# whatshap/whatshap

Measured on AMD Instinct MI355X. Metric: variant-columns/sec at max-coverage 20 (bipartition-costs/sec reported alongside), higher is better.
Workload: dtype u32; 1 GPU; synthetic diploid single-individual, max-coverage 20: 1 block of 200000 SNVs (BASELINE configs[2]); blocks=1, blocks_in_flight_per_gpu=1, tables_per_launch=1, max_coverage=20, optimal_cost_checksum=1611545, rendezvous=none

## Files before the change

whatshap_amd/csrc/dp_device.hip:

```cpp
#include <hip/hip_runtime.h>

#include <algorithm>
#include <atomic>
#include <cctype>
#include <chrono>
#include <cstdio>
#include <cstdlib>
#include <cstring>
#include <mutex>
#include <string>
#include <vector>

#include "debug_build.h"
#ifdef WHAMD_DEBUG_BUILD
#include "../../include/whatshap_amd_debug.h"
#endif
#include "device_runtime.h"
#include "device_table.h"
#include "genotype.h"
#include "table_plan.h"

namespace whamd {

namespace {
// ... 1567 lines not shown
		return WHAMD_OK;
	}
};

whamd_status_t DeviceTable::enqueue_group(DeviceTable* const* tables, const Problem* const* problems, Solution* const* solutions, size_t n_tables, std::string& msg) {
	if (n_tables == 0) return WHAMD_OK;
	HIP_TRY(hipSetDevice(tables[0]->impl_->device));
	Impl::GroupSubmission g(tables, problems, solutions, n_tables, msg);
	whamd_status_t st = g.open_members();
	if (st != WHAMD_OK) return st;
	const auto t_submit0 = std::chrono::steady_clock::now();
	for (size_t k = 0; k < g.max_steps; ++k) {
		g.add_super_step(k);
		for (int v = 0; v < GROUP_VARIANTS; ++v) g.flush((GroupVariant)v);
		if ((st = g.submit_singles(k)) != WHAMD_OK) return st;
	}
	if (getenv("WHAMD_DEBUG_TIMING"))
		fprintf(stderr, "[whamd timing] group of %zu tables in 1 part(s): %zu super-steps submitted in %.2f ms (host)\n", n_tables, g.max_steps,
		        std::chrono::duration<double, std::milli>(std::chrono::steady_clock::now() - t_submit0).count());
	if ((st = g.mark_forward_end()) != WHAMD_OK) return st;
	if ((st = g.walk_back()) != WHAMD_OK) return st;
	return g.submit_tails();
}

void DeviceTable::wait_last_of_each_stream(DeviceTable* const* tables, size_t n_tables) {
	std::vector<std::pair<hipStream_t, const Impl*>> last;
	for (size_t i = 0; i < n_tables; ++i) {
		const Impl& m = *tables[i]->impl_;
		if (!m.inflight.tail_elsewhere || !m.ev3) continue;
		bool found = false;
		for (auto& e : last) {
			if (e.first != m.inflight.tail_stream || e.second->device != m.device) continue;
			found = true;
			if (m.inflight.tail_seq > e.second->inflight.tail_seq) e.second = &m;
		}
		if (!found) last.emplace_back(m.inflight.tail_stream, &m);
	}
	for (const auto& e : last) {
		if (hipSetDevice(e.second->device) != hipSuccess || hipEventSynchronize(e.second->ev3) != hipSuccess) (void)hipGetLastError();
	}
}

void DeviceTable::read_timing(whamd_solve_stats& st) {
	Impl& m = *impl_;
	if (!m.inflight.timing_pending) return;
	m.inflight.timing_pending = false;
	if (hipSetDevice(m.device) != hipSuccess) return;
	float f01 = 0, f12 = 0, f03 = 0;
	if (hipEventElapsedTime(&f01, m.ev0, m.ev1) != hipSuccess || hipEventElapsedTime(&f12, m.ev1, m.ev2) != hipSuccess || hipEventElapsedTime(&f03, m.ev0, m.ev3) != hipSuccess) {
		(void)hipGetLastError();
		return;
	}
	st.forward_ms = f01;
	st.backtrace_ms = f12;
	st.total_ms = f03;
}

whamd_status_t DeviceTable::Impl::report_slot_stamps(std::string& msg) const {
	const Impl& m = *this;
	if (m.dev.dp.dbg_flags & 256u) return m.report_slot_wave_stamps(msg);
	std::vector<unsigned long long> d(m.tp.splan.runs.size() * 48);
	HIP_TRY(hipMemcpy(d.data(), m.dev.dp.dbg, d.size() * 8, hipMemcpyDeviceToHost));
	double a[6] = {0, 0, 0, 0, 0, 0};
	double percol[32] = {0};
	size_t cnt = 0;
	for (size_t i = 0; i < m.tp.splan.runs.size(); ++i) {
		if (m.tp.splan.runs[i].ncols != 22 || d[48 * i + 5] == 0) continue;
		for (int k = 0; k < 6; ++k) a[k] += (double)d[48 * i + k];
		for (int k = 0; k < 22; ++k) percol[k] += (double)d[48 * i + 8 + k];
		++cnt;
	}
	if (cnt) fprintf(stderr, "[whamd slot stamps] %zu runs, wave 0 of workgroup 0, shader cycles: prologue issue %.0f, loads landed %.0f, column loop %.0f (%.1f per column, %.1f columns), exit %.0f\n",
	                 cnt, a[0] / cnt, a[1] / cnt, a[2] / cnt, a[2] / std::max(a[4], 1.0), a[4] / cnt, a[3] / cnt);
	if (cnt) {
		fprintf(stderr, "[whamd slot stamps] cycles after the loop start at which column c had its cost added:");
		for (int k = 0; k < 22; ++k) fprintf(stderr, " %.0f", percol[k] / cnt);
		fprintf(stderr, "\n");
	}
	return WHAMD_OK;
}

whamd_status_t DeviceTable::Impl::report_slot_wave_stamps(std::string& msg) const {
	const Impl& m = *this;
	constexpr int NW = 8, NS = 8;
	static const char* const names[NS] = {"wave start", "entering cells requested", "last prologue request", "entering cells landed", "all landed, loop starts",
	                                      "first wave-slot ending reached", "first wave-slot ending left", "loop end"};
	static const int word[NS] = {0, 1, 2, 3, 7, 4, 5, 6};
	const size_t nruns = m.tp.splan.runs.size(), per_run = (size_t)SLOT_WAVE_STAMP_WGS * SLOT_WAVE_STAMP_WORDS;
	std::vector<unsigned long long> d(nruns * per_run);
	HIP_TRY(hipMemcpy(d.data(), m.dev.dp.dbg + m.dev.dp.dbg_wg_off + SLOT_WAVE_STAMP_OFF, d.size() * 8, hipMemcpyDeviceToHost));
	for (uint32_t sel = 0; sel < SLOT_WAVE_STAMP_WGS; ++sel) {
		double mean[NS][NW] = {}, spread[NS] = {}, spread_max[NS] = {}, lat_rank[NW] = {}, req_rank[NW] = {}, land_rank[NW] = {};
		size_t last[2][NW] = {}, cnt = 0;
		for (size_t i = 0; i < nruns; ++i) {
			const unsigned long long* r = d.data() + i * per_run + sel * SLOT_WAVE_STAMP_WORDS;
			bool full = m.tp.splan.runs[i].ncols == 22;
			for (int v = 0; v < NW; ++v) full = full && r[v * 8 + 6] != 0 && r[v * 8 + 4] != 0;
			if (!full) continue;
			unsigned long long s0 = r[0];
			for (int v = 1; v < NW; ++v) s0 = std::min(s0, r[v * 8]);
			double at[NS][NW];
			for (int k = 0; k < NS; ++k) {
				double lo = 1e300, hi = 0;
				int hi_at = 0;
				for (int v = 0; v < NW; ++v) {
					at[k][v] = (double)(r[v * 8] - s0) + (k ? (double)r[v * 8 + word[k]] : 0.0);
					mean[k][v] += at[k][v];
					lo = std::min(lo, at[k][v]);
					if (at[k][v] > hi) { hi = at[k][v]; hi_at = v; }
				}
				spread[k] += hi - lo;
				spread_max[k] = std::max(spread_max[k], hi - lo);
				if (k == 3) last[0][hi_at]++;
				if (k == 5) last[1][hi_at]++;
			}
			int order[NW];
			for (int v = 0; v < NW; ++v) order[v] = v;
			std::sort(order, order + NW, [&](int a, int b) { return at[1][a] < at[1][b]; });
			for (int q = 0; q < NW; ++q) { req_rank[q] += at[1][order[q]]; land_rank[q] += at[3][order[q]]; lat_rank[q] += at[3][order[q]] - at[1][order[q]]; }
			++cnt;
		}
		if (!cnt) continue;
		fprintf(stderr, "[whamd slot wave stamps] workgroup %u: %zu runs of 22 columns, shader cycles after the workgroup's earliest wave start; waves 0 .. 7 | mean spread, largest spread\n", 3 * sel, cnt);
		for (int k = 0; k < NS; ++k) {
			fprintf(stderr, "[whamd slot wave stamps]   %-31s", names[k]);
			for (int v = 0; v < NW; ++v) fprintf(stderr, " %6.0f", mean[k][v] / cnt);
			fprintf(stderr, " | %6.0f %6.0f\n", spread[k] / cnt, spread_max[k]);
		}
		for (int h = 0; h < 2; ++h) {
			fprintf(stderr, "[whamd slot wave stamps]   runs in which wave v is the last %-14s", h ? "at the ending:" : "to have cells:");
			for (int v = 0; v < NW; ++v) fprintf(stderr, " %6zu", last[h][v]);
			fprintf(stderr, "\n");
		}
		fprintf(stderr, "[whamd slot wave stamps]   by the order of the waves' requests -- requested:     ");
		for (int q = 0; q < NW; ++q) fprintf(stderr, " %6.0f", req_rank[q] / cnt);
		fprintf(stderr, "\n[whamd slot wave stamps]                                           landed:        ");
		for (int q = 0; q < NW; ++q) fprintf(stderr, " %6.0f", land_rank[q] / cnt);
		fprintf(stderr, "\n[whamd slot wave stamps]                                           latency:       ");
		for (int q = 0; q < NW; ++q) fprintf(stderr, " %6.0f", lat_rank[q] / cnt);
		fprintf(stderr, "\n");
	}
	return WHAMD_OK;
}

whamd_status_t DeviceTable::Impl::report_resident_stamps(std::string& msg) const {
	const Impl& m = *this;
	std::vector<unsigned long long> d(m.tp.plan.segments.size() * 8);
	HIP_TRY(hipMemcpy(d.data(), m.dev.dp.dbg, d.size() * 8, hipMemcpyDeviceToHost));
	unsigned long long a = 0, b = 0, c2 = 0, cols = 0, p1 = 0, p2 = 0, p3 = 0, ns = 0;
	for (size_t i = 0; i < m.tp.plan.segments.size(); ++i) { a += d[8 * i]; b += d[8 * i + 1]; c2 += d[8 * i + 2]; cols += d[8 * i + 3]; p1 += d[8 * i + 4]; p2 += d[8 * i + 5]; p3 += d[8 * i + 6]; ns += d[8 * i + 7]; }
	if (!m.tp.plan.ped_columns.empty() || (m.dev.dp.dbg_flags & 4u))
		fprintf(stderr, "[whamd timing] run prologue (wave 0 of workgroup 0), cycles after the first instruction: kernel arguments usable %.0f, first loaded data %.0f, everything staged %.0f\n",
		        (double)p2 / std::max<unsigned long long>(ns, 1), (double)p3 / std::max<unsigned long long>(ns, 1), (double)p1 / std::max<unsigned long long>(ns, 1));
	else
	fprintf(stderr, "[whamd timing] per barrier step (wave 0 of workgroup 0, %.1f steps per run): hot words %.0f, evaluate %.0f, barrier %.0f cycles\n",
	        (double)ns / m.tp.plan.segments.size(), (double)p1 / std::max<unsigned long long>(ns, 1), (double)p2 / std::max<unsigned long long>(ns, 1), (double)p3 / std::max<unsigned long long>(ns, 1));
	{
		unsigned long long b3[6] = {0, 0, 0, 0, 0, 0};
		HIP_TRY(hipMemcpy(b3, m.dev.dp.dbg + m.dev.dp.dbg_wg_off + 4 * 512 * 2, sizeof b3, hipMemcpyDeviceToHost));
		if (b3[2]) fprintf(stderr, "[whamd timing] backtrace per run: record load + prefetch %.0f cycles, walk + hand-over %.0f cycles (%llu runs); of the latter: local exit index %.0f, chain %.0f, logical indices + stores %.0f\n",
		                   (double)b3[0] / b3[2], (double)b3[1] / b3[2], b3[2], (double)b3[3] / b3[2], (double)b3[4] / b3[2], (double)b3[5] / b3[2]);
	}
	if (m.tp.plan.segments.size() > 104) {
		std::vector<unsigned long long> wg(4 * 512 * 2);
		HIP_TRY(hipMemcpy(wg.data(), m.dev.dp.dbg + m.dev.dp.dbg_wg_off, wg.size() * 8, hipMemcpyDeviceToHost));
		unsigned long long prev_end = 0;
		for (int sgi = 0; sgi < 4; ++sgi) {
			const uint32_t G = 1u << m.tp.plan.segments[100 + sgi].g;
			unsigned long long s0 = ~0ull, s1 = 0, e0 = ~0ull, e1 = 0;
			for (uint32_t ww = 0; ww < G; ++ww) {
				const unsigned long long a2 = wg[((size_t)sgi * 512 + ww) * 2], b2 = wg[((size_t)sgi * 512 + ww) * 2 + 1];
				s0 = std::min(s0, a2); s1 = std::max(s1, a2); e0 = std::min(e0, b2); e1 = std::max(e1, b2);
			}
			fprintf(stderr, "[whamd timing] run %d (%u workgroups): first start +%.2f us after previous run's last end; starts spread %.2f us; first end %.2f us, last end %.2f us after first start\n",
			        100 + sgi, G, prev_end ? (double)(s0 - prev_end) / 100.0 : 0.0, (double)(s1 - s0) / 100.0, (double)(e0 - s0) / 100.0, (double)(e1 - s0) / 100.0);
			prev_end = e1;
		}
	}
	float f01 = 0;
	(void)hipEventElapsedTime(&f01, m.ev0, m.ev1);
	fprintf(stderr, "[whamd timing] segments %zu cols %llu | cycles/segment: prologue %.0f columns %.0f (%.0f per column) store %.0f | fwd %.3f ms, %.2f us per segment\n",
	        m.tp.plan.segments.size(), cols, (double)a / m.tp.plan.segments.size(), (double)b / m.tp.plan.segments.size(),
	        (double)b / std::max<unsigned long long>(cols, 1), (double)c2 / m.tp.plan.segments.size(), f01, f01 * 1e3 / m.tp.plan.segments.size());
	return WHAMD_OK;
}

whamd_status_t DeviceTable::wait(const Problem& p, Solution& s, whamd_solve_stats& st, std::string& msg) {
	Impl& m = *impl_;
	if (p.n_cols == 0) return WHAMD_OK;
	HIP_TRY(hipSetDevice(m.device));
	const uint64_t launches = m.inflight.launches;
	if (m.inflight.tail_elsewhere) HIP_TRY(hipEventSynchronize(m.ev3));
	else { HIP_TRY(hipStreamSynchronize(m.stream)); m.own_stream_used = false; }
	m.upload_pending = false;
	m.give_preview_block();
	const uint32_t n = p.n_cols;
	std::memcpy(s.path_index.data(), m.dev.h_pinned, (size_t)n * 4);
// ... 202 lines not shown
```

whatshap_amd/csrc/kernels_slots.h:

```cpp

__device__ __forceinline__ uint32_t slot_cost(uint32_t A, uint32_t K, uint32_t Cc) { return min(min(A, K - A), Cc); }

template <int LR, int J>
__device__ __forceinline__ uint32_t slot_end_reg(uint32_t (&D)[1 << LR], uint32_t qthr, uint32_t qmask) {
	constexpr int R = 1 << LR;
	uint32_t takes = 0;
#pragma unroll
	for (int r0 = 0; r0 < R; ++r0) {
		if (r0 & (1 << J)) continue;
		const int r1 = r0 | (1 << J);
		const uint32_t q0 = qthr ^ ((qmask >> r0) & 1u), q1 = qthr ^ ((qmask >> r1) & 1u);
		const uint32_t a = D[r0], b = D[r1];
		takes |= (b < a + q0) ? (1u << r0) : 0u;
		takes |= (a < b + q1) ? (1u << r1) : 0u;
		D[r0] = D[r1] = min(a, b);
	}
	return takes;
}

template <int LR>
__device__ __forceinline__ uint32_t slot_end_partner(uint32_t (&D)[1 << LR], const uint32_t (&other)[1 << LR], uint32_t qthr, uint32_t qmask) {
	constexpr int R = 1 << LR;
	uint32_t takes = 0;
#pragma unroll
// ... 407 lines not shown
	"s_lshl_b32 %[sa], 1, %[sl]\n\t"                \
	"v_xor_b32_e32 %[a], %[sa], %[l4]\n\t"                                                                             \
	"ds_bpermute_b32 v60, %[a], %[d0]\n\t"                                                                             \
	"ds_bpermute_b32 v61, %[a], %[d1]\n\t"                                                                             \
	"ds_bpermute_b32 v62, %[a], %[d2]\n\t"                                                                             \
	"ds_bpermute_b32 v63, %[a], %[d3]\n\t"                                                                             \
	"s_branch .Lxm%=\n"                                                                                                \
	".Lxw%=:\n\t"                                   \
	"s_sub_u32 %[sa], %[sl], 8\n\t"                                                                                    \
	"s_lshl_b32 %[sa], 0x400, %[sa]\n\t"                                                                               \
	"s_bfe_u32 %[sl], %[cw], 0x1000f\n\t"           \
	"s_mul_i32 %[sl], %[sl], %[xby]\n\t"                                                                               \
	"v_mov_b32_e32 v56, %[d0]\n\t"                                                                                     \
	"v_mov_b32_e32 v57, %[d1]\n\t"                                                                                     \
	"v_mov_b32_e32 v58, %[d2]\n\t"                                                                                     \
	"v_mov_b32_e32 v59, %[d3]\n\t"                                                                                     \
	"v_add_u32_e32 %[a], %[sl], %[t16]\n\t"                                                                            \
	"ds_write_b128 %[a], v[56:59]\n\t"                                                                                 \
	"v_xor_b32_e32 %[a], %[sa], %[t16]\n\t"                                                                            \
	"v_add_u32_e32 %[a], %[sl], %[a]\n\t"                                                                              \
	"s_waitcnt lgkmcnt(0)\n\t"                                                                                         \
	"s_barrier\n\t"                                                                                                    \
	"ds_read_b128 v[60:63], %[a]\n\t"                                                                                  \
	"s_branch .Lxm%=\n"                                                                                                \
	".Lxr%=:\n\t"                                               \
	"s_cmp_eq_u32 %[sl], 0\n\t"                                                                                        \
	"s_cbranch_scc0 .Lxq%=\n\t"                                                                                        \
	"v_mov_b32_e32 v60, %[d1]\n\t"                                                                                     \
	"v_mov_b32_e32 v61, %[d0]\n\t"                                                                                     \
	"v_mov_b32_e32 v62, %[d3]\n\t"                                                                                     \
	"v_mov_b32_e32 v63, %[d2]\n\t"                                                                                     \
	"s_branch .Lxm%=\n"                                                                                                \
	".Lxq%=:\n\t"                                                                                                      \
	"v_mov_b32_e32 v60, %[d2]\n\t"                                                                                     \
	"v_mov_b32_e32 v61, %[d3]\n\t"                                                                                     \
	"v_mov_b32_e32 v62, %[d0]\n\t"                                                                                     \
	"v_mov_b32_e32 v63, %[d1]\n"                                                                                       \
	".Lxm%=:\n\t"                                   \
	"v_and_b32_e32 %[t], 1, %[par]\n\t"                                                                                \
	"v_cmp_ne_u32_e64 %[qt], 0, %[t]\n\t"                                                                              \
	"v_lshrrev_b32_e32 %[par], 1, %[par]\n\t"                             \
	"s_not_b64 %[qn], %[qt]\n\t"                                                                                       \
	"s_bitcmp1_b32 %[cw], 8\n\t"                     \
	"s_cselect_b64 %[q1], %[qn], %[qt]\n\t"                                                                            \
	"s_bitcmp1_b32 %[cw], 9\n\t"                                                                                       \
	"s_cselect_b64 %[q2], %[qn], %[qt]\n\t"                                                                            \
	"s_bitcmp1_b32 %[cw], 10\n\t"                                                                                      \
	"s_cselect_b64 %[q3], %[qn], %[qt]\n\t"                                                                            \
	"s_waitcnt lgkmcnt(0)\n\t"                                                                                         \
	"v_subb_co_u32_e64 %[t], %[q3], %[d3], v63, %[q3]\n\t"                                                                     \
	"v_subb_co_u32_e64 %[t], %[q2], %[d2], v62, %[q2]\n\t"                                                             \
	"v_subb_co_u32_e64 %[t], %[q1], %[d1], v61, %[q1]\n\t"                                                             \
	"v_subb_co_u32_e64 %[t], %[qt], %[d0], v60, %[qt]\n\t"                                                             \
	"v_cndmask_b32_e64 %[tk], 0, 1, %[q3]\n\t"                                                                         \
	"v_max_u32_e32 %[d3], %[d3], v63\n\t"                                                                              \
	"v_addc_co_u32_e64 %[tk], %[qn], %[tk], %[tk], %[q2]\n\t"                                                          \
	"v_max_u32_e32 %[d2], %[d2], v62\n\t"                                                                              \
	"v_addc_co_u32_e64 %[tk], %[qn], %[tk], %[tk], %[q1]\n\t"                                                          \
	"v_max_u32_e32 %[d1], %[d1], v61\n\t"                                                                              \
	"v_addc_co_u32_e64 %[tk], %[qn], %[tk], %[tk], %[qt]\n\t"                                                          \
	"v_max_u32_e32 %[d0], %[d0], v60\n\t"                                                                              \
	"global_store_byte %[ro], %[tk], %[rb]\n\t"     \
	"v_add_u32_e32 %[ro], %[thr], %[ro]"

#define SLOT_TOUCH_1(o) "s_load_dword %0, %1, " #o "\n\t"
#define SLOT_TOUCH_4(a, b, c, d) SLOT_TOUCH_1(a) SLOT_TOUCH_1(b) SLOT_TOUCH_1(c) SLOT_TOUCH_1(d)
template <int N>
__device__ __forceinline__ uint32_t slot_touch_lines(const void* base) {
	static_assert(N == 2 || N == 4 || N == 8 || N == 12 || N == 16, "touch counts that are written out");
	uint32_t junk;
	const unsigned long long b = (unsigned long long)base;
	if (N == 2) asm volatile(SLOT_TOUCH_1(64) SLOT_TOUCH_1(128) : "=s"(junk) : "s"(b) : "memory");
	if (N == 4) asm volatile(SLOT_TOUCH_4(64, 128, 192, 256) : "=s"(junk) : "s"(b) : "memory");
	if (N == 8) asm volatile(SLOT_TOUCH_4(64, 128, 192, 256) SLOT_TOUCH_4(320, 384, 448, 512) : "=s"(junk) : "s"(b) : "memory");
	if (N == 12) asm volatile(SLOT_TOUCH_4(64, 128, 192, 256) SLOT_TOUCH_4(320, 384, 448, 512) SLOT_TOUCH_4(576, 640, 704, 768) : "=s"(junk) : "s"(b) : "memory");
	if (N == 16) asm volatile(SLOT_TOUCH_4(64, 128, 192, 256) SLOT_TOUCH_4(320, 384, 448, 512) SLOT_TOUCH_4(576, 640, 704, 768) SLOT_TOUCH_4(832, 896, 960, 1024) : "=s"(junk) : "s"(b) : "memory");
	return junk;
}
__device__ __forceinline__ void slot_touch_done(uint32_t junk) { asm volatile("" ::"s"(junk)); }

struct SlotxStamps {
	unsigned long long t_start, t_issued, t_loaded, t_loop;
	uint32_t w_enter = 0, w_landed = 0, w_end_in = 0, w_end_out = 0;
};
constexpr uint32_t SLOT_WAVE_STAMP_WGS = 3, SLOT_WAVE_STAMP_WORDS = 8 * 8, SLOT_WAVE_STAMP_OFF = 4 * 512 * 2 + 16;
__device__ __forceinline__ bool slot_wave_stamps_on(const DevProblem& P) { return P.dbg && (P.dbg_flags & 256u); }
template <int LR, int XC, bool DBG>
__device__ __forceinline__ void slot_runx_core(const DevProblem& P, const SlotRun& run, const uint32_t* __restrict__ prev, const uint32_t w, uint32_t (&D)[1 << LR],
                                               SlotxStamps& stamps, const void* warm = nullptr) {
	static_assert(LR == 2, "X runs: four cells per thread (the masks, the decisions and the exchange are written for four)");
	static_assert(XC % 4 == 0 && XC <= SLOT_XCOLS, "whole trips of four columns");
	constexpr bool STREAM = XC == 0;
	constexpr int R = 1 << LR;
	extern __shared__ __attribute__((aligned(16))) uint32_t smem[];
	const unsigned long long t_start = (DBG && P.dbg) ? __builtin_readcyclecounter() : 0ull;
	const uint32_t tid = threadIdx.x, lane = tid & 63u;
	const uint32_t wave = uni(tid >> 6);
	if (!STREAM && wave >= 4u) __builtin_amdgcn_s_setprio(1);
	const uint32_t L = run.L;
	const uint32_t lthr = tid << LR;
	const uint32_t Pthr = (w << L) | lthr;
	const uint32_t ncols = run.ncols, threads = run.threads;
	const uint32_t ncp = (ncols + 7u) & ~7u;
	const uint32_t* __restrict__ tab = P.slot_tab;
	const uint32_t* __restrict__ kr_tab = tab + run.tab_kr;
	const uint32_t* __restrict__ cw_tab = kr_tab + ((ncols + (uint32_t)SLOT_XPAD) << LR);
	typedef uint32_t slot_u32x4c __attribute__((ext_vector_type(4)));
	typedef const __attribute__((address_space(4))) slot_u32x4c* slot_cptr4c;
	slot_u32x16 krA = *(slot_cptr16)(unsigned long long)kr_tab, krB;
	slot_u32x4c cwA = *(slot_cptr4c)(unsigned long long)cw_tab, cwB;
	const uint32_t par_w = *(const __attribute__((address_space(4))) uint32_t*)(unsigned long long)(tab + run.tab_par + threads + w);
	uint32_t touch_kr = 0, touch_kr2 = 0, touch_cw = 0, touch_g = 0, touch_w = 0;
	uint32_t warm_junk = 0;
	if (warm) {
		const unsigned long long line = (unsigned long long)warm + ((lane & 7u) << 6);
		asm volatile("global_load_dword %0, %1, off" : "=v"(warm_junk) : "v"(line) : "memory");
	}
	uint32_t Draw[R];
	bool flip;
	slot_enter_cells<LR, DBG>(P, run, prev, Pthr, Draw, flip);
	const bool wstamps = DBG && slot_wave_stamps_on(P);
	if (DBG && wstamps) asm volatile("" ::: "memory");
	stamps.w_enter = (DBG && wstamps) ? (uint32_t)__builtin_readcyclecounter() : 0u;
	if (DBG && wstamps) asm volatile("" ::: "memory");
	const uint32_t par_l = tab[run.tab_par + tid];
	const uint32_t* __restrict__ sl_src = tab + run.tab_sl + lane;
	const uint32_t* __restrict__ g_row = tab + run.tab_g + w * ncp;
	const uint32_t* __restrict__ w_row = tab + run.tab_w + wave * ncp;
	typedef uint32_t slot_u32x4s __attribute__((ext_vector_type(4)));
	typedef const __attribute__((address_space(4))) slot_u32x4s* slot_cptr4;
	slot_u32x4s gA, gB, wA, wB;
	uint32_t slA[4], slB[4];
	unsigned long long t_issued = 0ull;
	if (STREAM) {
		gA = *(slot_cptr4)(unsigned long long)g_row;
		wA = *(slot_cptr4)(unsigned long long)w_row;
#pragma unroll
		for (int k = 0; k < 4; ++k) slA[k] = sl_src[64 * k];
		touch_kr = slot_touch_lines<8>(kr_tab);
		touch_cw = slot_touch_lines<2>(cw_tab);
		touch_g = slot_touch_lines<2>(g_row);
		touch_w = slot_touch_lines<2>(w_row);
		t_issued = (DBG && P.dbg) ? __builtin_readcyclecounter() : 0ull;
		if (DBG && wstamps) asm volatile("s_waitcnt vmcnt(5)" ::: "memory");
		stamps.w_landed = (DBG && wstamps) ? (uint32_t)__builtin_readcyclecounter() : 0u;
	} else {
		const uint32_t cl = lane < ncols ? lane : 0u;
		const uint32_t a_g = g_row[cl], a_w = w_row[cl];
		uint32_t X[XC > 0 ? XC : 4];
#pragma unroll
		for (int c = 0; c < XC; ++c) X[c] = sl_src[64 * c];
		touch_kr = slot_touch_lines<(XC <= 8 ? 4 : 8)>(kr_tab);
		if (XC > 24) touch_kr2 = slot_touch_lines<2>(kr_tab + 128);
		touch_cw = slot_touch_lines<2>(cw_tab);
		t_issued = (DBG && P.dbg) ? __builtin_readcyclecounter() : 0ull;
		if (DBG && wstamps) asm volatile("s_waitcnt vmcnt(%0)" ::"n"(XC + 3) : "memory");
		stamps.w_landed = (DBG && wstamps) ? (uint32_t)__builtin_readcyclecounter() : 0u;
		const uint32_t Avec = lane < ncols ? a_g + a_w : 0u;
		uint4* __restrict__ xs = reinterpret_cast<uint4*>(smem + 2u * threads * R) + tid;
#pragma unroll
		for (int t4 = 0; t4 < XC / 4; ++t4) {
			uint32_t x[4];
#pragma unroll
			for (int k = 0; k < 4; ++k) x[k] = X[4 * t4 + k] + (uint32_t)__builtin_amdgcn_readlane((int)Avec, 4 * t4 + k);
			xs[(uint32_t)t4 * threads] = make_uint4(x[0], x[1], x[2], x[3]);
		}
	}
	uint32_t par = par_l ^ par_w;
	uint8_t* __restrict__ rec = P.bt + (((unsigned long long)run.rec_hi << 32) | run.rec_lo) + (size_t)w * run.n_ends * threads;
#pragma unroll
	for (int r = 0; r < R; ++r) D[r] = flip ? Draw[R - 1 - r] : Draw[r];
	if (!(run.yflags & 2u)) {
#pragma unroll
		for (int r = 0; r < R; ++r) D[r] = run.base_in - 2u * D[r];
	}
	if (warm) asm volatile("" ::"v"(warm_junk), "v"(D[0]));
	if (DBG && P.dbg) asm volatile("s_waitcnt vmcnt(0)" ::: "memory");
	const unsigned long long t_loaded = (DBG && P.dbg) ? __builtin_readcyclecounter() + (D[0] & 0u) : 0ull;
	if (!STREAM) __builtin_amdgcn_s_setprio(0);

	const uint32_t lds0 = (uint32_t)(unsigned long long)smem;
	const uint32_t lane4 = lane << 2, tid16 = lds0 + (tid << 4);
	const uint32_t xbytes = threads * R * 4u;
	uint32_t rec_off = tid;
	const SlotRow* __restrict__ rows = P.slot_rows + run.row_off;
	auto ending = [&](const uint32_t field) {
		unsigned long long q1, q2, q3, qt, qn;
		uint32_t t, a, sa, sl, takes;
		asm volatile(SLOTX_ENDING_ASM
		             : [d0] "+v"(D[0]), [d1] "+v"(D[1]), [d2] "+v"(D[2]), [d3] "+v"(D[3]), [par] "+v"(par), [ro] "+v"(rec_off), [tk] "=&v"(takes), [t] "=&v"(t), [a] "=&v"(a),
		               [sa] "=&s"(sa), [sl] "=&s"(sl), [q1] "=&s"(q1), [q2] "=&s"(q2), [q3] "=&s"(q3), [qt] "=&s"(qt), [qn] "=&s"(qn)
		             : [cw] "s"(field), [xby] "s"(xbytes), [thr] "s"(threads), [rb] "s"(rec), [l4] "v"(lane4), [t16] "v"(tid16)
		             : "memory", "scc", "v56", "v57", "v58", "v59", "v60", "v61", "v62", "v63");
	};
	uint32_t ci = 0;
	auto column = [&](const uint32_t x, const uint32_t k0, const uint32_t k1, const uint32_t k2, const uint32_t k3, const uint32_t ctrl) {
		D[0] = slot_y_sad_s(x, k0, D[0]);
		D[1] = slot_y_sad_s(x, k1, D[1]);
		D[2] = slot_y_sad_s(x, k2, D[2]);
		D[3] = slot_y_sad_s(x, k3, D[3]);
		if (DBG && P.dbg && !wstamps && w == 0 && tid == 0 && ci < 32u) P.dbg[(size_t)run.pad * 48 + 8 + ci] = __builtin_readcyclecounter() - t_loaded;
		if (ctrl & 3u) {
			if (DBG && wstamps && !stamps.w_end_in && ((ctrl >> 2) & 31u) >= 8u) {
				stamps.w_end_in = (uint32_t)__builtin_readcyclecounter() | 1u;
				ending(ctrl);
				stamps.w_end_out = (uint32_t)__builtin_readcyclecounter() + (D[0] & 0u);
			} else {
				ending(ctrl);
			}
			if (ctrl & 2u) {
				const unsigned long long row = (unsigned long long)(rows + ci);
				uint32_t n_end = 2u, info = 0u;
				if (ctrl & 1u) {
					n_end = *(const __attribute__((address_space(4))) uint32_t*)(row + 44);
					info = *(const __attribute__((address_space(4))) uint32_t*)(row + 64);
				}
				ending(ctrl >> 16);
				for (uint32_t e = 2; e < n_end; ++e) {
					const uint32_t field = ((info & 31u) << 2) | (((info >> 8) & 15u) << 7) | (((info >> 16) & 1u) << 15);
					if (e + 1u < n_end) info = *(const __attribute__((address_space(4))) uint32_t*)(row + 56 + 8 * e);
					ending(field);
				}
			}
		}
		++ci;
	};
	if (STREAM) {
		{
			asm volatile("" ::"s"(krA[0]), "s"(cwA[0]), "s"(gA[0]), "s"(wA[0]));
			slot_touch_done(touch_kr); slot_touch_done(touch_cw); slot_touch_done(touch_g); slot_touch_done(touch_w);
		}
		for (uint32_t pairs = (ncols + 7u) >> 3; pairs; --pairs) {
			asm volatile("" ::"s"(krA[0]), "s"(cwA[0]), "s"(gA[0]), "s"(wA[0]));
			krB = *(slot_cptr16)(unsigned long long)(kr_tab + 16u);
			cwB = *(slot_cptr4c)(unsigned long long)(cw_tab + 4u);
			gB = *(slot_cptr4)(unsigned long long)(g_row + 4u);
			wB = *(slot_cptr4)(unsigned long long)(w_row + 4u);
#pragma unroll
			for (int k = 0; k < 4; ++k) slB[k] = sl_src[64 * (4 + k)];
			column(slA[0] + (gA[0] + wA[0]), krA[0], krA[1], krA[2], krA[3], cwA[0]);
			column(slA[1] + (gA[1] + wA[1]), krA[4], krA[5], krA[6], krA[7], cwA[1]);
			column(slA[2] + (gA[2] + wA[2]), krA[8], krA[9], krA[10], krA[11], cwA[2]);
			column(slA[3] + (gA[3] + wA[3]), krA[12], krA[13], krA[14], krA[15], cwA[3]);
			asm volatile("" ::"s"(krB[0]), "s"(cwB[0]), "s"(gB[0]), "s"(wB[0]));
			kr_tab += 32u;
			cw_tab += 8u;
			g_row += 8u;
			w_row += 8u;
			sl_src += 512u;
			krA = *(slot_cptr16)(unsigned long long)kr_tab;
			cwA = *(slot_cptr4c)(unsigned long long)cw_tab;
			gA = *(slot_cptr4)(unsigned long long)g_row;
			wA = *(slot_cptr4)(unsigned long long)w_row;
#pragma unroll
			for (int k = 0; k < 4; ++k) slA[k] = sl_src[64 * k];
			column(slB[0] + (gB[0] + wB[0]), krB[0], krB[1], krB[2], krB[3], cwB[0]);
			column(slB[1] + (gB[1] + wB[1]), krB[4], krB[5], krB[6], krB[7], cwB[1]);
			column(slB[2] + (gB[2] + wB[2]), krB[8], krB[9], krB[10], krB[11], cwB[2]);
			column(slB[3] + (gB[3] + wB[3]), krB[12], krB[13], krB[14], krB[15], cwB[3]);
		}
	} else {
// ... 183 lines not shown
		asm volatile(SLOTX8_ENDING_ASM
		             : [d0] "+v"(D[0]), [d1] "+v"(D[1]), [d2] "+v"(D[2]), [d3] "+v"(D[3]), [d4] "+v"(D[4]), [d5] "+v"(D[5]), [d6] "+v"(D[6]), [d7] "+v"(D[7]), [par] "+v"(par),
		               [ro] "+v"(rec_off), [tk] "=&v"(takes), [t] "=&v"(t), [sa] "=&s"(sa), [sl] "=&s"(sl), [q1] "=&s"(q1), [q2] "=&s"(q2), [q3] "=&s"(q3), [q4] "=&s"(q4),
		               [q5] "=&s"(q5), [q6] "=&s"(q6), [q7] "=&s"(q7), [qt] "=&s"(qt), [qn] "=&s"(qn)
		             : [cw] "s"(field), [xby] "s"(xbytes), [thr] "s"(threads), [rb] "s"(rec), [l4] "v"(lane4), [t32] "v"(tid32)
		             : "memory", "scc", "v48", "v49", "v50", "v51", "v52", "v53", "v54", "v55", "v56", "v57", "v58", "v59", "v60", "v61", "v62", "v63");
	};
	uint32_t ci = 0;
	auto column = [&](const uint32_t x, const slot_u32x16& kr, const int half, const uint32_t ctrl) {
#pragma unroll
		for (int r = 0; r < R; ++r) D[r] = slot_y_sad_s(x, kr[half * 8 + r], D[r]);
		if (DBG && P.dbg && w == 0 && tid == 0 && ci < 32u) P.dbg[(size_t)run.pad * 48 + 8 + ci] = __builtin_readcyclecounter() - t_loaded;
		if (ctrl & 3u) {
			ending(ctrl);
			if (ctrl & 2u) {
				const unsigned long long row = (unsigned long long)(rows + ci);
				uint32_t n_end = 2u, info = 0u;
				if (ctrl & 1u) {
					n_end = *(slot_cptr1)(row + 44);
					info = *(slot_cptr1)(row + 64);
				}
				ending(ctrl >> 16);
				for (uint32_t e = 2; e < n_end; ++e) {
					const uint32_t field = ((info & 31u) << 2) | (((info >> 8) & 255u) << 7) | (((info >> 16) & 1u) << 15);
					if (e + 1u < n_end) info = *(slot_cptr1)(row + 56 + 8 * e);
					ending(field);
				}
			}
		}
		++ci;
	};
	{
		asm volatile("" ::"s"(krA[0]), "s"(cwA[0]), "s"(gA[0]), "s"(wA[0]));
		slot_touch_done(touch_kr); slot_touch_done(touch_cw); slot_touch_done(touch_g); slot_touch_done(touch_w);
	}
	for (uint32_t quads = (ncols + 3u) >> 2; quads; --quads) {
		asm volatile("" ::"s"(krA[0]), "s"(cwA[0]), "s"(gA[0]), "s"(wA[0]));
		krB = *(slot_cptr16)(unsigned long long)(kr_tab + 16u);
		cwB = *(slot_cptr2)(unsigned long long)(cw_tab + 2u);
		gB = *(slot_cptr2)(unsigned long long)(g_row + 2u);
		wB = *(slot_cptr2)(unsigned long long)(w_row + 2u);
		slB[0] = sl_src[128];
		slB[1] = sl_src[192];
		column(slA[0] + (gA[0] + wA[0]), krA, 0, cwA[0]);
		column(slA[1] + (gA[1] + wA[1]), krA, 1, cwA[1]);
		asm volatile("" ::"s"(krB[0]), "s"(cwB[0]), "s"(gB[0]), "s"(wB[0]));
		kr_tab += 32u;
		cw_tab += 4u;
		g_row += 4u;
		w_row += 4u;
		sl_src += 256u;
		krA = *(slot_cptr16)(unsigned long long)kr_tab;
		cwA = *(slot_cptr2)(unsigned long long)cw_tab;
		gA = *(slot_cptr2)(unsigned long long)g_row;
		wA = *(slot_cptr2)(unsigned long long)w_row;
		slA[0] = sl_src[0];
		slA[1] = sl_src[64];
		column(slB[0] + (gB[0] + wB[0]), krB, 0, cwB[0]);
		column(slB[1] + (gB[1] + wB[1]), krB, 1, cwB[1]);
	}
	stamps.t_start = t_start; stamps.t_issued = t_issued; stamps.t_loaded = t_loaded;
	stamps.t_loop = (DBG && P.dbg) ? __builtin_readcyclecounter() + (D[0] & 0u) : 0ull;
}

template <int LR, bool DBG, bool SPEC>
__device__ __forceinline__ void slot_runx_exit(const DevProblem& P, const SlotRun& run, uint32_t* __restrict__ cur, uint32_t* score_out, const uint32_t w, uint32_t (&D)[1 << LR],
                                               const SlotxStamps& stamps) {
	const uint32_t tid = threadIdx.x, lane = tid & 63u;
	const uint32_t wave = uni(tid >> 6);
	const uint32_t L = run.L, lthr = tid << LR;
	slot_exit_cells<LR, DBG, SPEC, true>(P, run, cur, D, w, tid, lane, wave, L, lthr, (w << L) | lthr, run.threads);
	if (score_out && w == 0 && tid == 0) *score_out = D[0];
	if (DBG && P.dbg && w == 0 && tid == 0) {
		unsigned long long* d = P.dbg + (size_t)run.pad * 48;
		d[0] = stamps.t_issued - stamps.t_start; d[1] = stamps.t_loaded - stamps.t_start; d[2] = stamps.t_loop - stamps.t_loaded; d[3] = __builtin_readcyclecounter() - stamps.t_loop;
		d[4] = run.ncols; d[5] = 1;
	}
	if (DBG && slot_wave_stamps_on(P) && lane == 0 && w < 3u * SLOT_WAVE_STAMP_WGS && w % 3u == 0u) {
		unsigned long long* d = P.dbg + P.dbg_wg_off + SLOT_WAVE_STAMP_OFF + ((size_t)run.pad * SLOT_WAVE_STAMP_WGS + w / 3u) * SLOT_WAVE_STAMP_WORDS + wave * 8u;
		const uint32_t t0 = (uint32_t)stamps.t_start;
		d[0] = stamps.t_start;
		d[1] = stamps.w_enter - t0; d[2] = (uint32_t)stamps.t_issued - t0; d[3] = stamps.w_landed - t0;
		d[4] = stamps.w_end_in ? (stamps.w_end_in - t0) : 0u; d[5] = stamps.w_end_in ? (stamps.w_end_out - t0) : 0u; d[6] = (uint32_t)stamps.t_loop - t0;
		d[7] = (uint32_t)stamps.t_loaded - t0;
	}
}
template <int LR, int XC, bool DBG, bool SPEC>
__device__ __forceinline__ void slot_runx_body(const DevProblem& P, const SlotRun& run, const uint32_t* __restrict__ prev, uint32_t* __restrict__ cur, const uint32_t w,
                                               uint32_t* score_out) {
	uint32_t D[1 << LR];
	SlotxStamps stamps;
	slot_runx_core<LR, XC, DBG>(P, run, prev, w, D, stamps);
	slot_runx_exit<LR, DBG, SPEC>(P, run, cur, score_out, w, D, stamps);
}

__global__ __launch_bounds__(256) void slot_tables(DevProblem P, const SlotRun* __restrict__ runs, uint32_t* __restrict__ tab) {
	const SlotRun& run = runs[blockIdx.y];
	const uint32_t ncols = run.ncols, L = run.L, lr = run.lr, nwg = 1u << (run.g - run.half), nwaves = run.threads >> 6;
	const uint32_t ncp = (run.yflags & 8u) ? (ncols + 7u) & ~7u : ncols;
	const uint32_t n_g = nwg * ncp, n_w = nwaves * ncp, n_sl = ncp * 64u;
	const bool xrun = (run.yflags & 8u) != 0u;
	const uint32_t R = 1u << lr, n_krw = xrun ? (ncols + (uint32_t)SLOT_XPAD) * R : 0u, n_kr = xrun ? n_krw + ncols + (uint32_t)SLOT_XPAD : 0u, n_par = xrun ? run.threads + nwg : 0u;
	const SlotRow* __restrict__ rows = P.slot_rows + run.row_off;
	const uint32_t ysh = run.yflags & 1u, ybias = ysh ? SLOT_YBIAS : 0u;
	for (uint32_t i = blockIdx.x * blockDim.x + threadIdx.x; i < n_g + n_w + n_sl + n_kr + n_par; i += gridDim.x * blockDim.x) {
		if (i >= n_g + n_w + n_sl + n_kr) {
			const uint32_t q = i - (n_g + n_w + n_sl + n_kr);
			const uint32_t index = q < run.threads ? (q << lr) : ((q - run.threads) << L);
			const uint32_t keep = q < run.threads ? (1u << L) - 1u : ~((1u << L) - 1u);
			uint32_t bits = 0, e = 0;
			for (uint32_t c = 0; c < ncols; ++c) {
				const uint32_t n_end = rows[c].n_end;
				for (uint32_t k = 0; k < n_end; ++k, ++e) bits |= ((uint32_t)__popc(index & keep & rows[c].end[k].M) & 1u) << (e & 31u);
			}
			tab[run.tab_par + q] = bits;
		} else if (i >= n_g + n_w + n_sl + n_krw) {
			const uint32_t c = i - (n_g + n_w + n_sl + n_krw);
			uint32_t word = 0;
			if (c < ncols) {
				const SlotRow& row = rows[c];
				auto field = [](uint32_t info) { return ((info & 31u) << 2) | (((info >> 8) & 255u) << 7) | (((info >> 16) & 1u) << 15); };
				if (row.n_end) word = (row.n_end < 3u ? row.n_end : 3u) | field(row.end[0].info);
				if (row.n_end > 1u) word |= field(row.end[1].info) << 16;
			}
			tab[run.tab_kr + n_krw + c] = word;
		} else if (i >= n_g + n_w + n_sl) {
			const uint32_t q = i - (n_g + n_w + n_sl), c = q / R, r = q % R;
			tab[run.tab_kr + q] = c < ncols ? reinterpret_cast<const uint32_t*>(rows + c)[r] : 0u;
		} else if (i < n_g) {
			const uint32_t w = i / ncp, c = i % ncp;
			const SlotRow& row = rows[c < ncols ? c : 0u];
			uint32_t acc = row.Cp;
			for (uint32_t s = L; s < L + run.g; ++s) acc += (uint32_t)row.dslot[s] & (0u - ((w >> (s - L)) & 1u));
			tab[run.tab_g + i] = c < ncols ? (acc << ysh) + ybias : 0u;
		} else if (i < n_g + n_w) {
			const uint32_t q = i - n_g, wave = q / ncp, c = q % ncp;
			const SlotRow& row = rows[c < ncols ? c : 0u];
			uint32_t acc = 0;
			for (uint32_t s = lr + 6u; s < L; ++s) acc += (uint32_t)row.dslot[s] & (0u - ((wave >> (s - lr - 6u)) & 1u));
			tab[run.tab_w + q] = c < ncols ? acc << ysh : 0u;
		} else {
			const uint32_t q = i - n_g - n_w, c = q >> 6, lane = q & 63u;
			const SlotRow& row = rows[c < ncols ? c : 0u];
			uint32_t acc = 0;
			for (uint32_t j = 0; j < (uint32_t)SLOT_LANE; ++j) acc += (uint32_t)row.dslot[lr + j] & (0u - ((lane >> j) & 1u));
			tab[run.tab_sl + q] = c < ncols ? acc << ysh : 0u;
		}
	}
}

template <int LR, int XC, bool DBG, bool SPEC>
__global__ __launch_bounds__(512) void slot_runx(DevProblem P, SlotRun run, const uint32_t* __restrict__ prev, uint32_t* __restrict__ cur, uint32_t* __restrict__ score_out,
                                                 uint32_t pack) {
	if (pack && (blockIdx.x & 7u)) return;
	touch_kernel_arguments<sizeof(DevProblem) + sizeof(SlotRun) + 28>();
	slot_runx_body<LR, XC, DBG, SPEC>(P, run, prev, cur, pack ? blockIdx.x >> 3 : blockIdx.x, score_out);
}

template <int LR, bool DBG, bool SPEC, bool YF = false>
__global__ __launch_bounds__(512) void slot_run(DevProblem P, SlotRun run, const uint32_t* __restrict__ prev, uint32_t* __restrict__ cur,
                                                uint32_t* __restrict__ score_out) {
	touch_kernel_arguments<sizeof(DevProblem) + sizeof(SlotRun) + 24>();
	slot_run_body<LR, DBG, SPEC, YF>(P, run, prev, cur, blockIdx.x, score_out);
}

template <int LR>
__global__ __launch_bounds__(512) void slot_batch(DevProblem P, const SlotBatchEntry* __restrict__ entries) {
	const SlotBatchEntry* __restrict__ e = entries + blockIdx.y;
	{
		const uint32_t* lines = reinterpret_cast<const uint32_t*>(e);
		uint32_t acc = 0;
#pragma unroll
		for (uint32_t l = 0; l < (sizeof(SlotBatchEntry) + 63) / 64; ++l) acc |= lines[l * 16];
		asm volatile("" ::"s"(__builtin_amdgcn_readfirstlane(acc)));
	}
	const SlotRun run = e->run;
	if (blockIdx.x >= (1u << (run.g - run.half)) || threadIdx.x >= run.threads) return;
	if ((LR == 2 || LR == 3) && (run.yflags & 1u)) slot_run_body<(LR == 3 ? 3 : 2), false, false, true>(P, run, e->prev, e->cur, blockIdx.x, e->score_out);
	else slot_run_body<LR, false, false>(P, run, e->prev, e->cur, blockIdx.x, e->score_out);
}

template <class T>
__device__ __forceinline__ T slot_scalar_copy(const T* __restrict__ p) {
	static_assert(sizeof(T) % 4 == 0, "whole words");
	T out;
	uint32_t* w = reinterpret_cast<uint32_t*>(&out);
	const __attribute__((address_space(4))) uint32_t* src = (const __attribute__((address_space(4))) uint32_t*)(unsigned long long)p;
#pragma unroll
	for (uint32_t i = 0; i < sizeof(T) / 4; ++i) w[i] = src[i];
	return out;
}

__device__ __forceinline__ DevProblem slot_entry_problem(const SlotBatchEntry& e, bool ped) {
	DevProblem P{};
	if (ped) { P.pslot_tab = e.tab; P.pslot_rows = reinterpret_cast<const PedSlotRow*>(e.rows); }
	else { P.slot_tab = e.tab; P.slot_rows = reinterpret_cast<const SlotRow*>(e.rows); }
	P.slot_ctrl = e.ctrl;
	P.bt = e.bt;
	P.spec_keys = e.spec_keys;
	P.spec_stride = e.spec_stride;
	return P;
}

__device__ __forceinline__ uint32_t slot_warm_next(const SlotBatchEntry* ep) {
	uint32_t junk;
	const unsigned long long line = (unsigned long long)(ep + 1) + ((threadIdx.x & 7u) << 6);
	asm volatile("global_load_dword %0, %1, off" : "=v"(junk) : "v"(line) : "memory");
	return junk;
}
__device__ __forceinline__ void slot_warm_done(uint32_t junk) { asm volatile("" ::"v"(junk)); }

struct SlotGroupWho { uint32_t table, w; bool none; };
__device__ __forceinline__ SlotGroupWho slot_group_who(const SlotGroupArgs& args) {
	SlotGroupWho who;
	who.table = args.pad ? blockIdx.x : blockIdx.y;
	who.w = args.pad ? blockIdx.y : blockIdx.x;
	who.none = who.table >= args.n;
	return who;
}

template <int LR = 2, bool DBG = false>
__global__ __launch_bounds__(512, 4) void slot_groupx(SlotGroupArgs args) {
	const SlotGroupWho who = slot_group_who(args);
	if (who.none) return;
	const SlotBatchEntry* ep = args.entry[who.table];
	uint32_t D[1 << LR];
	SlotxStamps stamps;
	{
		const SlotBatchEntry e = slot_scalar_copy(ep);
		if (who.w >= (1u << (e.run.g - e.run.half)) || threadIdx.x >= e.run.threads) return;
		DevProblem P = slot_entry_problem(e, false);
		if (DBG) P.dbg_flags = e.pad2;
		const void* warm = (e.pad2 & 0x10000u) ? nullptr : (const void*)(ep + 1);
		if constexpr (LR == 3) slot_runx8_core<DBG>(P, e.run, e.prev, who.w, D, stamps, warm);
		else slot_runx_core<2, 0, DBG>(P, e.run, e.prev, who.w, D, stamps, warm);
	}
	asm volatile("" : "+s"(ep));
	const SlotBatchEntry e = slot_scalar_copy(ep);
	DevProblem P = slot_entry_problem(e, false);
// ... 22 lines not shown
```

Measured before the change: 2.400 million variant-columns/s.

## Hand-schedule kernel argument loads and defer scalar table loads in X slot runs

For non-streaming X runs, the kernel now fetches its arguments with one hand-ordered block of scalar loads and raises the priority of the upper waves inside the same asm. Loading the kr/cw/parity scalar tables is moved after the entering-cell loads, so the vector loads are issued first. The flip swap becomes a ballot mask driving inline v_cndmask instructions. A debug stamp for when the scalar tables land is added. The aim is to shorten the per-run prologue latency, at the cost of fragile inline asm that depends on struct offsets.

```diff
diff --git a/whatshap_amd/csrc/dp_device.hip b/whatshap_amd/csrc/dp_device.hip
--- a/whatshap_amd/csrc/dp_device.hip
+++ b/whatshap_amd/csrc/dp_device.hip
@@ -1673,10 +1673,11 @@
 
 whamd_status_t DeviceTable::Impl::report_slot_wave_stamps(std::string& msg) const {
 	const Impl& m = *this;
-	constexpr int NW = 8, NS = 8;
+	constexpr int NW = 8, NS = 9;
 	static const char* const names[NS] = {"wave start", "entering cells requested", "last prologue request", "entering cells landed", "all landed, loop starts",
-	                                      "first wave-slot ending reached", "first wave-slot ending left", "loop end"};
-	static const int word[NS] = {0, 1, 2, 3, 7, 4, 5, 6};
+	                                      "scalar tables landed too", "first wave-slot ending reached", "first wave-slot ending left", "loop end"};
+	static const int word[NS] = {0, 1, 2, 3, 7, 8, 4, 5, 6};
+	auto stamp = [](const unsigned long long* wave_words, int k) { return k == 8 ? wave_words[7] >> 32 : (k == 7 ? wave_words[7] & 0xFFFFFFFFull : wave_words[k]); };
 	const size_t nruns = m.tp.splan.runs.size(), per_run = (size_t)SLOT_WAVE_STAMP_WGS * SLOT_WAVE_STAMP_WORDS;
 	std::vector<unsigned long long> d(nruns * per_run);
 	HIP_TRY(hipMemcpy(d.data(), m.dev.dp.dbg + m.dev.dp.dbg_wg_off + SLOT_WAVE_STAMP_OFF, d.size() * 8, hipMemcpyDeviceToHost));
@@ -1695,7 +1696,7 @@
 				double lo = 1e300, hi = 0;
 				int hi_at = 0;
 				for (int v = 0; v < NW; ++v) {
-					at[k][v] = (double)(r[v * 8] - s0) + (k ? (double)r[v * 8 + word[k]] : 0.0);
+					at[k][v] = (double)(r[v * 8] - s0) + (k ? (double)stamp(r + v * 8, word[k]) : 0.0);
 					mean[k][v] += at[k][v];
 					lo = std::min(lo, at[k][v]);
 					if (at[k][v] > hi) { hi = at[k][v]; hi_at = v; }
@@ -1703,7 +1704,7 @@
 				spread[k] += hi - lo;
 				spread_max[k] = std::max(spread_max[k], hi - lo);
 				if (k == 3) last[0][hi_at]++;
-				if (k == 5) last[1][hi_at]++;
+				if (k == 6) last[1][hi_at]++;
 			}
 			int order[NW];
 			for (int v = 0; v < NW; ++v) order[v] = v;
diff --git a/whatshap_amd/csrc/kernels_slots.h b/whatshap_amd/csrc/kernels_slots.h
--- a/whatshap_amd/csrc/kernels_slots.h
+++ b/whatshap_amd/csrc/kernels_slots.h
@@ -513,6 +513,7 @@
 struct SlotxStamps {
 	unsigned long long t_start, t_issued, t_loaded, t_loop;
 	uint32_t w_enter = 0, w_landed = 0, w_end_in = 0, w_end_out = 0;
+	uint32_t w_scalars = 0;
 };
 constexpr uint32_t SLOT_WAVE_STAMP_WGS = 3, SLOT_WAVE_STAMP_WORDS = 8 * 8, SLOT_WAVE_STAMP_OFF = 4 * 512 * 2 + 16;
 __device__ __forceinline__ bool slot_wave_stamps_on(const DevProblem& P) { return P.dbg && (P.dbg_flags & 256u); }
@@ -527,21 +528,33 @@
 	const unsigned long long t_start = (DBG && P.dbg) ? __builtin_readcyclecounter() : 0ull;
 	const uint32_t tid = threadIdx.x, lane = tid & 63u;
 	const uint32_t wave = uni(tid >> 6);
-	if (!STREAM && wave >= 4u) __builtin_amdgcn_s_setprio(1);
 	const uint32_t L = run.L;
 	const uint32_t lthr = tid << LR;
 	const uint32_t Pthr = (w << L) | lthr;
 	const uint32_t ncols = run.ncols, threads = run.threads;
 	const uint32_t ncp = (ncols + 7u) & ~7u;
 	const uint32_t* __restrict__ tab = P.slot_tab;
-	const uint32_t* __restrict__ kr_tab = tab + run.tab_kr;
-	const uint32_t* __restrict__ cw_tab = kr_tab + ((ncols + (uint32_t)SLOT_XPAD) << LR);
+	const uint32_t* __restrict__ kr_tab;
+	const uint32_t* __restrict__ cw_tab;
 	typedef uint32_t slot_u32x4c __attribute__((ext_vector_type(4)));
 	typedef const __attribute__((address_space(4))) slot_u32x4c* slot_cptr4c;
-	slot_u32x16 krA = *(slot_cptr16)(unsigned long long)kr_tab, krB;
-	slot_u32x4c cwA = *(slot_cptr4c)(unsigned long long)cw_tab, cwB;
-	const uint32_t par_w = *(const __attribute__((address_space(4))) uint32_t*)(unsigned long long)(tab + run.tab_par + threads + w);
+	slot_u32x16 krA, krB;
+	slot_u32x4c cwA, cwB;
+	uint32_t par_w;
 	uint32_t touch_kr = 0, touch_kr2 = 0, touch_cw = 0, touch_g = 0, touch_w = 0;
+	auto request_tables = [&]() {
+		kr_tab = tab + run.tab_kr;
+		cw_tab = kr_tab + ((ncols + (uint32_t)SLOT_XPAD) << LR);
+		krA = *(slot_cptr16)(unsigned long long)kr_tab;
+		cwA = *(slot_cptr4c)(unsigned long long)cw_tab;
+		par_w = *(const __attribute__((address_space(4))) uint32_t*)(unsigned long long)(tab + run.tab_par + threads + w);
+		if (!STREAM) {
+			touch_kr = slot_touch_lines<(XC <= 8 ? 4 : 8)>(kr_tab);
+			if (XC > 24) touch_kr2 = slot_touch_lines<2>(kr_tab + 128);
+			touch_cw = slot_touch_lines<2>(cw_tab);
+		}
+	};
+	if (STREAM) request_tables();
 	uint32_t warm_junk = 0;
 	if (warm) {
 		const unsigned long long line = (unsigned long long)warm + ((lane & 7u) << 6);
@@ -550,6 +563,8 @@
 	uint32_t Draw[R];
 	bool flip;
 	slot_enter_cells<LR, DBG>(P, run, prev, Pthr, Draw, flip);
+	unsigned long long fmask = __builtin_amdgcn_ballot_w64(flip);
+	asm volatile("" : "+s"(fmask));
 	const bool wstamps = DBG && slot_wave_stamps_on(P);
 	if (DBG && wstamps) asm volatile("" ::: "memory");
 	stamps.w_enter = (DBG && wstamps) ? (uint32_t)__builtin_readcyclecounter() : 0u;
@@ -581,9 +596,7 @@
 		uint32_t X[XC > 0 ? XC : 4];
 #pragma unroll
 		for (int c = 0; c < XC; ++c) X[c] = sl_src[64 * c];
-		touch_kr = slot_touch_lines<(XC <= 8 ? 4 : 8)>(kr_tab);
-		if (XC > 24) touch_kr2 = slot_touch_lines<2>(kr_tab + 128);
-		touch_cw = slot_touch_lines<2>(cw_tab);
+		request_tables();
 		t_issued = (DBG && P.dbg) ? __builtin_readcyclecounter() : 0ull;
 		if (DBG && wstamps) asm volatile("s_waitcnt vmcnt(%0)" ::"n"(XC + 3) : "memory");
 		stamps.w_landed = (DBG && wstamps) ? (uint32_t)__builtin_readcyclecounter() : 0u;
@@ -599,8 +612,13 @@
 	}
 	uint32_t par = par_l ^ par_w;
 	uint8_t* __restrict__ rec = P.bt + (((unsigned long long)run.rec_hi << 32) | run.rec_lo) + (size_t)w * run.n_ends * threads;
-#pragma unroll
-	for (int r = 0; r < R; ++r) D[r] = flip ? Draw[R - 1 - r] : Draw[r];
+	asm("s_nop 1\n\t"
+	    "v_cndmask_b32_e64 %0, %4, %7, %8\n\t"
+	    "v_cndmask_b32_e64 %1, %5, %6, %8\n\t"
+	    "v_cndmask_b32_e64 %2, %6, %5, %8\n\t"
+	    "v_cndmask_b32_e64 %3, %7, %4, %8"
+	    : "=&v"(D[0]), "=&v"(D[1]), "=&v"(D[2]), "=&v"(D[3])
+	    : "v"(Draw[0]), "v"(Draw[1]), "v"(Draw[2]), "v"(Draw[3]), "s"(fmask));
 	if (!(run.yflags & 2u)) {
 #pragma unroll
 		for (int r = 0; r < R; ++r) D[r] = run.base_in - 2u * D[r];
@@ -608,6 +626,9 @@
 	if (warm) asm volatile("" ::"v"(warm_junk), "v"(D[0]));
 	if (DBG && P.dbg) asm volatile("s_waitcnt vmcnt(0)" ::: "memory");
 	const unsigned long long t_loaded = (DBG && P.dbg) ? __builtin_readcyclecounter() + (D[0] & 0u) : 0ull;
+	if (DBG && wstamps) asm volatile("s_waitcnt lgkmcnt(0)" ::: "memory");
+	stamps.w_scalars = (DBG && wstamps) ? (uint32_t)__builtin_readcyclecounter() : 0u;
+	if (DBG && wstamps) asm volatile("" ::: "memory");
 	if (!STREAM) __builtin_amdgcn_s_setprio(0);
 
 	const uint32_t lds0 = (uint32_t)(unsigned long long)smem;
@@ -957,7 +978,7 @@
 		d[0] = stamps.t_start;
 		d[1] = stamps.w_enter - t0; d[2] = (uint32_t)stamps.t_issued - t0; d[3] = stamps.w_landed - t0;
 		d[4] = stamps.w_end_in ? (stamps.w_end_in - t0) : 0u; d[5] = stamps.w_end_in ? (stamps.w_end_out - t0) : 0u; d[6] = (uint32_t)stamps.t_loop - t0;
-		d[7] = (uint32_t)stamps.t_loaded - t0;
+		d[7] = (unsigned long long)((uint32_t)stamps.t_loaded - t0) | ((unsigned long long)(stamps.w_scalars ? stamps.w_scalars - t0 : 0u) << 32);
 	}
 }
 template <int LR, int XC, bool DBG, bool SPEC>
@@ -1024,12 +1045,81 @@
 	}
 }
 
+struct SlotRunxArgs {
+	DevProblem P;
+	SlotRun run;
+	const uint32_t* prev;
+	uint32_t* cur;
+	uint32_t* score_out;
+	uint32_t pack;
+};
+__device__ __forceinline__ void slot_runx_arguments(SlotRunxArgs& a) {
+	typedef const __attribute__((address_space(4))) void* karg_ptr;
+	const karg_ptr ka = (karg_ptr)__builtin_amdgcn_kernarg_segment_ptr();
+	const uint32_t tid0 = uni(threadIdx.x);
+	constexpr uint32_t RUN = sizeof(DevProblem), TAIL = sizeof(DevProblem) + sizeof(SlotRun);
+	static_assert(offsetof(SlotRun, in_fullmask) == 64 && offsetof(SlotRun, spec_id) == 80 && offsetof(SlotRun, out_pos) == 128 && offsetof(SlotRun, tab_g) == 160 &&
+	              sizeof(SlotRun) == 192 && sizeof(DevProblem) % 8 == 0, "the word groups below");
+	unsigned long long bt, rows, tab, keys, prev, cur, score;
+	uint32_t stride, pack;
+	slot_u32x16 r0;
+	slot_u32x4 r16, r20;
+	slot_u32x8 r32, r40;
+	asm volatile(
+	    "s_load_dwordx16 %[r0], %[ka], %[o_run]\n\t"
+	    "s_load_dwordx2 %[prev], %[ka], %[o_tail]\n\t"
+	    "s_load_dwordx2 %[tab], %[ka], %[o_tab]\n\t"
+	    "s_load_dwordx8 %[r40], %[ka], %[o_run] + 160\n\t"
+	    "s_load_dwordx4 %[r16], %[ka], %[o_run] + 64\n\t"
+	    "s_load_dword %[pack], %[ka], %[o_tail] + 24\n\t"
+	    "s_load_dwordx4 %[r20], %[ka], %[o_run] + 80\n\t"
+	    "s_load_dwordx8 %[r32], %[ka], %[o_run] + 128\n\t"
+	    "s_load_dwordx2 %[cur], %[ka], %[o_tail] + 8\n\t"
+	    "s_load_dwordx2 %[score], %[ka], %[o_tail] + 16\n\t"
+	    "s_load_dwordx2 %[bt], %[ka], %[o_bt]\n\t"
+	    "s_load_dwordx2 %[rows], %[ka], %[o_rows]\n\t"
+	    "s_load_dwordx2 %[keys], %[ka], %[o_keys]\n\t"
+	    "s_load_dword %[stride], %[ka], %[o_stride]\n\t"
+	    "s_cmpk_lt_u32 %[tid0], 0x100\n\t"
+	    "s_cbranch_scc1 .Lxa%=\n\t"
+	    "s_setprio 1\n"
+	    ".Lxa%=:\n\t"
+	    "s_waitcnt lgkmcnt(0)"
+	    : [r0] "=&s"(r0), [r16] "=&s"(r16), [r20] "=&s"(r20), [r32] "=&s"(r32), [r40] "=&s"(r40), [bt] "=&s"(bt), [rows] "=&s"(rows), [tab] "=&s"(tab), [keys] "=&s"(keys),
+	      [stride] "=&s"(stride), [prev] "=&s"(prev), [cur] "=&s"(cur), [score] "=&s"(score), [pack] "=&s"(pack)
+	    : [ka] "s"(ka), [tid0] "s"(tid0), [o_run] "n"(RUN), [o_tail] "n"(TAIL), [o_bt] "n"(offsetof(DevProblem, bt)), [o_rows] "n"(offsetof(DevProblem, slot_rows)),
+	      [o_tab] "n"(offsetof(DevProblem, slot_tab)), [o_keys] "n"(offsetof(DevProblem, spec_keys)), [o_stride] "n"(offsetof(DevProblem, spec_stride))
+	    : "memory", "scc");
+	a.P = DevProblem{};
+	auto global = [](unsigned long long v, auto* type) { return (decltype(type))(__attribute__((address_space(1))) void*)v; };
+	a.P.bt = global(bt, (uint8_t*)nullptr); a.P.slot_rows = global(rows, (const SlotRow*)nullptr); a.P.slot_tab = global(tab, (const uint32_t*)nullptr);
+	a.P.spec_keys = global(keys, (unsigned long long*)nullptr); a.P.spec_stride = stride;
+	uint32_t* rw = reinterpret_cast<uint32_t*>(&a.run);
+#pragma unroll
+	for (int i = 0; i < 16; ++i) rw[i] = r0[i];
+#pragma unroll
+	for (int i = 0; i < 4; ++i) { rw[16 + i] = r16[i]; rw[20 + i] = r20[i]; }
+#pragma unroll
+	for (int i = 0; i < 8; ++i) { rw[32 + i] = r32[i]; rw[40 + i] = r40[i]; }
+	a.prev = global(prev, (const uint32_t*)nullptr); a.cur = global(cur, (uint32_t*)nullptr); a.score_out = global(score, (uint32_t*)nullptr); a.pack = pack;
+}
+
 template <int LR, int XC, bool DBG, bool SPEC>
 __global__ __launch_bounds__(512) void slot_runx(DevProblem P, SlotRun run, const uint32_t* __restrict__ prev, uint32_t* __restrict__ cur, uint32_t* __restrict__ score_out,
                                                  uint32_t pack) {
-	if (pack && (blockIdx.x & 7u)) return;
-	touch_kernel_arguments<sizeof(DevProblem) + sizeof(SlotRun) + 28>();
-	slot_runx_body<LR, XC, DBG, SPEC>(P, run, prev, cur, pack ? blockIdx.x >> 3 : blockIdx.x, score_out);
+	if constexpr (XC == 0) {
+		if (pack && (blockIdx.x & 7u)) return;
+		touch_kernel_arguments<sizeof(DevProblem) + sizeof(SlotRun) + 28>();
+		slot_runx_body<LR, XC, DBG, SPEC>(P, run, prev, cur, pack ? blockIdx.x >> 3 : blockIdx.x, score_out);
+	} else {
+		SlotRunxArgs a;
+		slot_runx_arguments(a);
+#pragma unroll
+		for (int i = 0; i < 8; ++i) a.run.in_pos[i] = run.in_pos[i];
+		if (DBG) { a.P.dbg = P.dbg; a.P.dbg_wg_off = P.dbg_wg_off; a.P.dbg_flags = P.dbg_flags; }
+		if (a.pack && (blockIdx.x & 7u)) return;
+		slot_runx_body<LR, XC, DBG, SPEC>(a.P, a.run, a.prev, a.cur, a.pack ? blockIdx.x >> 3 : blockIdx.x, a.score_out);
+	}
 }
 
 template <int LR, bool DBG, bool SPEC, bool YF = false>
```

After: 2.466 million variant-columns/s (median of 6 runs). 1.03x the previous value.
